# deeppowers/deeppowers

Measured on AMD Instinct MI355X. Metric: ciphertext-mul/s (N=4096, 4 RNS limbs), higher is better.
Workload: dtype u64

## Files before the change

### deeppowers_amd/csrc/devtables.h

```cpp
#pragma once
#include "modarith.h"

namespace dpfhe {

struct QuartersTop;

template <class Tw>
struct InvLast {
    Tw w_last;
    Tw w_ninv;
};

template <class Arith>
struct DevTables {
    const typename Arith::Tw* fwd;
    const typename Arith::Tw* inv;
    const typename Arith::Tw* fwd4;
    const typename Arith::Tw* inv4;
    const typename Arith::Tw* top_fwd;
    const typename Arith::Tw* top_inv;
    const InvLast<typename Arith::Tw>* top_last;
    int n_sub;
    const typename Arith::Tw* hfwd;
    const typename Arith::Tw* hinv;
    const typename Arith::Tw* htop_fwd;
    const InvLast<typename Arith::Tw>* htop_last;
    const typename Arith::Tw* qfwd;
    const typename Arith::Tw* qinv;
    const struct QuartersTop* qtop_fwd;
    const typename Arith::Tw* qtop_inv;
    const InvLast<typename Arith::Tw>* qtop_last;
    const InvLast<typename Arith::Tw>* last;
    const InvLast<typename Arith::Tw>* last2;
    const LimbConst* lc;
    int n_limbs;
    int n_active;
    unsigned long long active_map;
};

template <class TB>
DPF_HD void block_item_limb(const TB& tb, size_t blk, size_t& item, int& limb) {
    if (tb.n_active) {
        item = blk / (unsigned)tb.n_active;
        limb = (int)((tb.active_map >> (4u * (unsigned)(blk % (unsigned)tb.n_active))) & 15u);
    } else {
        item = blk / (unsigned)tb.n_limbs;
        limb = (int)(blk % (unsigned)tb.n_limbs);
    }
}

struct MixedTables {
    const void* fwd;
    const void* inv;
    const void* last;
    const LimbConst* lc;
    int n_limbs;
// ... 5 lines not shown
```

### deeppowers_amd/csrc/dpfhe_cabi.hip

```cpp
#include <dlfcn.h>
#include <hip/hip_runtime.h>

#include <algorithm>
#include <atomic>
#include <cstdio>
#include <cstdlib>
#include <cstring>
#include <mutex>
#include <new>
#include <string>
#include <type_traits>
#include <vector>

#include "../../include/dpfhe.h"
#include "base_ext.h"
#include "expand.h"
#include "plain_add.h"
#include "kernels_large.h"
#include "kernels_misc.h"
#include "launch.h"
#include "ntt_core.h"
#include "ntt_quarters.h"
#include "tables.h"

// ... 177 lines not shown
    return DPFHE_SUCCESS;
}
extern "C" int dpfhe_ctx_tune_info(const dpfhe_ctx* c, dpfhe_tune_info* out) {
    if (!c || !out) return fail(DPFHE_INVALID_ARGUMENT, "dpfhe_ctx_tune_info", "null argument");
    std::lock_guard<std::mutex> lk(c->tune_mutex);
    *out = c->tune;
    out->chosen = c->ct_mul_variant.load();
    return DPFHE_SUCCESS;
}
extern "C" int dpfhe_ctx_set_ct_mul_variant(dpfhe_ctx* c, int variant) {
    if (!c) return fail(DPFHE_INVALID_ARGUMENT, "dpfhe_ctx_set_ct_mul_variant", "null context");
    if (!ct_mul_variant_compiled(c, variant)) return fail(DPFHE_INVALID_ARGUMENT, "dpfhe_ctx_set_ct_mul_variant", "this context has no such form of the fused multiply");
    std::lock_guard<std::mutex> lk(c->tune_mutex);
    c->ct_mul_variant.store(variant);
    c->tune.chosen = variant;
    c->tune.source = DPFHE_TUNE_FORCED;
    return DPFHE_SUCCESS;
}
extern "C" const char* dpfhe_ct_mul_variant_name(int variant) {
    return variant >= 0 && variant < kCtMulVariants ? kCtMulVariantNames[variant] : "";
}

static_assert(sizeof(TwShoup) == 16 && sizeof(TwFold) == 16 && sizeof(TwF64) == 16, "the per-limb slots of the mixed tables share one stride");
struct MixedLayout { size_t o_lc, o_fwd4, o_inv4, o_fwd, o_inv, o_last, o_last2, total; };
static MixedLayout mixed_layout(int log2n, size_t L) {
    auto up = [](size_t x) { return (x + 255) & ~(size_t)255; };
    const size_t n = (size_t)1 << log2n, tab = L * n * 16;
    const bool two_geo = ntt_loge(log2n) != kFusedLoge;
    MixedLayout m;
    m.o_lc = 0; m.o_fwd4 = up(L * sizeof(LimbConst)); m.o_inv4 = up(m.o_fwd4 + tab);
    m.o_fwd = two_geo ? up(m.o_inv4 + tab) : m.o_fwd4; m.o_inv = two_geo ? up(m.o_fwd + tab) : m.o_inv4;
    m.o_last = up(m.o_inv + tab); m.o_last2 = up(m.o_last + L * 32); m.total = up(m.o_last2 + L * 32);
    return m;
}
template <class Tw, class MakeTw>
static void fill_mixed_limb(std::vector<unsigned char>& blob, const MixedLayout& m, int log2n, size_t l, const HostLimbTables& t, LimbClass cls, MakeTw make_tw) {
    static_assert(sizeof(Tw) == 16 && sizeof(InvLast<Tw>) == 32, "slot sizes");
    const size_t n = (size_t)1 << log2n;
    const u64 q = t.lc.q;
    const LimbConst lc = limb_const_of_class(t.lc, cls);
    std::memcpy(&blob[m.o_lc + l * sizeof(LimbConst)], &lc, sizeof(LimbConst));
    auto pack = [&](const std::vector<u64>& words, int loge, size_t off) {
        std::vector<Tw> tw(words.size());
        for (size_t i = 0; i < words.size(); ++i) tw[i] = make_tw(words[i], q);
        permute_window0(tw, log2n, loge, geo_perm_stages(log2n, loge));
        std::memcpy(&blob[off], tw.data(), tw.size() * sizeof(Tw));
    };
    pack(t.rp, kFusedLoge, m.o_fwd4 + l * n * 16);
    pack(t.irp, kFusedLoge, m.o_inv4 + l * n * 16);
    if (m.o_fwd != m.o_fwd4) { pack(t.rp, ntt_loge(log2n), m.o_fwd + l * n * 16); pack(t.irp, ntt_loge(log2n), m.o_inv + l * n * 16); }
    reinterpret_cast<InvLast<Tw>*>(&blob[m.o_last])[l] = InvLast<Tw>{make_tw(t.w_last, q), make_tw(t.lc.ninv, q)};
    const u64 sinv = cls == kClassFoldScaled ? h_powmod((1ull << fold_scaled_shift(q)) % q, q - 2, q) : 1;
    reinterpret_cast<InvLast<Tw>*>(&blob[m.o_last2])[l] = InvLast<Tw>{make_tw(h_mulmod(t.w_last, sinv, q), q), make_tw(h_mulmod(t.lc.ninv, sinv, q), q)};
}
template <class Arith>
static DevTables<Arith> mixed_view(const unsigned char* b, const MixedLayout& m, size_t L) {
    typedef typename Arith::Tw Tw;
    DevTables<Arith> tb{};
    tb.lc = reinterpret_cast<const LimbConst*>(b + m.o_lc);
    tb.fwd = reinterpret_cast<const Tw*>(b + m.o_fwd); tb.inv = reinterpret_cast<const Tw*>(b + m.o_inv);
    tb.fwd4 = reinterpret_cast<const Tw*>(b + m.o_fwd4); tb.inv4 = reinterpret_cast<const Tw*>(b + m.o_inv4);
    tb.last = reinterpret_cast<const InvLast<Tw>*>(b + m.o_last);
    tb.last2 = reinterpret_cast<const InvLast<Tw>*>(b + m.o_last2);
    tb.n_sub = 1;
    tb.n_limbs = (int)L;
    return tb;
}

extern "C" int dpfhe_ctx_create(dpfhe_ctx** out, uint32_t log2_n, uint32_t n_limbs, const uint64_t* moduli,
                                const uint64_t* psi, int device_id) {
    if (!out || !moduli || !psi) return fail(DPFHE_INVALID_ARGUMENT, "dpfhe_ctx_create", "null argument");
    if (log2_n < 8 || log2_n > (uint32_t)kMaxLog2N) return fail(DPFHE_INVALID_ARGUMENT, "dpfhe_ctx_create", "log2_n must be in [8, 16]");
    if (n_limbs == 0 || n_limbs > 1024) return fail(DPFHE_INVALID_ARGUMENT, "dpfhe_ctx_create", "n_limbs must be in [1, 1024]");
    const size_t n = (size_t)1 << log2_n, L = n_limbs;
    std::vector<HostLimbTables> ht(L);
    bool fold = true;
    for (size_t l = 0; l < L; ++l) {
        if (!h_is_prime(moduli[l])) return fail(DPFHE_INVALID_ARGUMENT, "dpfhe_ctx_create", "modulus is not prime");
        int rc = build_limb_tables((int)log2_n, moduli[l], psi[l], ht[l]);
        if (rc) return fail(rc, "dpfhe_ctx_create", "modulus must be < 2^60 and 1 mod 2N, psi a primitive 2N-th root");
        fold = fold && fold_eligible(moduli[l]);
    }
    int ndev = 0;
    HIP_TRY(hipGetDeviceCount(&ndev));
    if (device_id < 0 || device_id >= ndev) return fail(DPFHE_INVALID_ARGUMENT, "dpfhe_ctx_create", "no such device");
    int prev = 0;
// ... 3 lines not shown
    dpfhe_ctx* c = new (std::nothrow) dpfhe_ctx;
    if (!c) return fail(DPFHE_OUT_OF_MEMORY, "dpfhe_ctx_create", "host allocation");
    c->log2n = log2_n; c->n_limbs = n_limbs; c->device = device_id; c->fold = fold; c->p_special = moduli[L - 1];
    c->moduli.assign(moduli, moduli + L);
    { int cus = 0; if (hipDeviceGetAttribute(&cus, hipDeviceAttributeMultiprocessorCount, device_id) == hipSuccess && cus > 0) c->n_cu = cus; }

    auto up = [](size_t x) { return (x + 255) & ~(size_t)255; };
    const size_t tw_sz = fold ? sizeof(TwFold) : sizeof(TwShoup);
    const int log_n1 = split_log_n1((int)log2_n), log_n2 = (int)log2_n - log_n1;
    const size_t n_sub = (size_t)1 << log_n1, n2 = (size_t)1 << log_n2;
    const int loge_ntt = ntt_loge(log_n2);
    const bool split = log_n1 > 0, two_geo = !split && loge_ntt != kFusedLoge;
    const size_t tab = L * n * tw_sz;
    const size_t o_lc = 0, o_fwd4 = up(o_lc + L * sizeof(LimbConst)), o_inv4 = up(o_fwd4 + tab),
                 o_fwd = two_geo ? up(o_inv4 + tab) : o_fwd4, o_inv = two_geo ? up(o_fwd + tab) : o_inv4,
                 o_last = up(o_inv + tab), o_top_fwd = up(o_last + L * n_sub * 2 * tw_sz), o_top_inv = up(o_top_fwd + L * n_sub * tw_sz),
                 o_top_last = up(o_top_inv + L * n_sub * tw_sz), o_resc = up(o_top_last + L * 2 * tw_sz);
    const bool halves = log2_n == 13 && fold;
    const size_t o_hfwd = up(o_resc + L * sizeof(RescaleConst)), o_hinv = halves ? up(o_hfwd + tab) : o_hfwd, o_htop_fwd = halves ? up(o_hinv + tab) : o_hfwd,
                 o_htop_last = halves ? up(o_htop_fwd + L * tw_sz) : o_hfwd, o_q0 = halves ? up(o_htop_last + L * 2 * tw_sz) : o_hfwd;
    const bool quarters = log2_n == 14 && fold;
    const size_t o_qfwd = o_q0, o_qinv = quarters ? up(o_qfwd + tab) : o_q0, o_qtop_fwd = quarters ? up(o_qinv + tab) : o_q0,
                 o_qtop_inv = quarters ? up(o_qtop_fwd + L * sizeof(QuartersTop)) : o_q0, o_qtop_last = quarters ? up(o_qtop_inv + L * 2 * tw_sz) : o_q0,
                 total = quarters ? up(o_qtop_last + L * 2 * tw_sz) : o_q0;
    std::vector<unsigned char> blob(total, 0);
    auto fill = [&](auto tw_tag) {
        typedef decltype(tw_tag) Tw;
        for (size_t l = 0; l < L; ++l) {
            const u64 q = moduli[l];
            auto pack = [&](const std::vector<u64>& words, int logn_tab, int loge, size_t off) {
                std::vector<Tw> t(words.size());
                for (size_t i = 0; i < words.size(); ++i) t[i] = h_make_tw<Tw>(words[i], q);
                permute_window0(t, logn_tab, loge, geo_perm_stages(logn_tab, loge));
                std::memcpy(&blob[off], t.data(), t.size() * sizeof(Tw));
            };
            InvLast<Tw>* lasts = reinterpret_cast<InvLast<Tw>*>(&blob[o_last]);
            if (!split) {
                for (int geo = 0; geo < (two_geo ? 2 : 1); ++geo) {
                    const int loge = geo ? loge_ntt : kFusedLoge;
                    pack(ht[l].rp, (int)log2_n, loge, (geo ? o_fwd : o_fwd4) + l * n * tw_sz);
                    pack(ht[l].irp, (int)log2_n, loge, (geo ? o_inv : o_inv4) + l * n * tw_sz);
                }
                lasts[l] = InvLast<Tw>{h_make_tw<Tw>(ht[l].w_last, q), h_make_tw<Tw>(ht[l].lc.ninv, q)};
                if constexpr (std::is_same<Tw, TwFold>::value) {
                    if (quarters) {
                        for (size_t r = 0; r < 4; ++r) {
                            pack(subtree_table(ht[l].rp, 14, 2, r), 12, 4, o_qfwd + (l * 4 + r) * (n / 4) * tw_sz);
                            pack(subtree_table(ht[l].irp, 14, 2, r), 12, 4, o_qinv + (l * 4 + r) * (n / 4) * tw_sz);
                        }
                        reinterpret_cast<QuartersTop*>(&blob[o_qtop_fwd])[l] = QuartersTop{h_tw_fold(ht[l].rp[1], q), h_tw_fold(ht[l].rp[2], q), h_tw_fold(ht[l].rp[3], q)};
                        reinterpret_cast<TwFold*>(&blob[o_qtop_inv])[2 * l] = h_tw_fold(ht[l].irp[2], q);
                        reinterpret_cast<TwFold*>(&blob[o_qtop_inv])[2 * l + 1] = h_tw_fold(ht[l].irp[3], q);
                        reinterpret_cast<InvLast<TwFold>*>(&blob[o_qtop_last])[l] = InvLast<TwFold>{h_tw_fold(ht[l].w_last, q), h_tw_fold(ht[l].lc.ninv, q)};
                    }
                }
                if (halves) {
                    for (size_t r = 0; r < 2; ++r) {
                        pack(subtree_table(ht[l].rp, 13, 1, r), 12, 4, o_hfwd + (l * 2 + r) * (n / 2) * tw_sz);
                        pack(subtree_table(ht[l].irp, 13, 1, r), 12, 4, o_hinv + (l * 2 + r) * (n / 2) * tw_sz);
                    }
                    reinterpret_cast<Tw*>(&blob[o_htop_fwd])[l] = h_make_tw<Tw>(ht[l].rp[1], q);
                    reinterpret_cast<InvLast<Tw>*>(&blob[o_htop_last])[l] = lasts[l];
                }
            } else {
                for (size_t r = 0; r < n_sub; ++r) {
                    const std::vector<u64> f = subtree_table(ht[l].rp, (int)log2_n, log_n1, r), v = subtree_table(ht[l].irp, (int)log2_n, log_n1, r);
                    pack(f, log_n2, loge_ntt, o_fwd + (l * n_sub + r) * n2 * tw_sz);
// ... 21 lines not shown
    }
    hipError_t e = hipMalloc(&c->d_blob, total);
    if (e == hipSuccess) e = hipMemcpy(c->d_blob, blob.data(), total, hipMemcpyHostToDevice);
    if (e != hipSuccess) {
        if (c->d_blob) (void)hipFree(c->d_blob);
        delete c;
        (void)hipSetDevice(prev);
        return fail(e == hipErrorOutOfMemory ? DPFHE_OUT_OF_MEMORY : DPFHE_DEVICE_ERROR, "dpfhe_ctx_create: table upload", hipGetErrorString(e));
    }
    unsigned char* d = static_cast<unsigned char*>(c->d_blob);
    c->d_rescale = reinterpret_cast<const RescaleConst*>(d + o_resc);
    if (fold) {
        c->foldt.lc = reinterpret_cast<const LimbConst*>(d + o_lc);
        c->foldt.fwd = reinterpret_cast<const TwFold*>(d + o_fwd);
        c->foldt.inv = reinterpret_cast<const TwFold*>(d + o_inv);
        c->foldt.fwd4 = reinterpret_cast<const TwFold*>(d + o_fwd4);
        c->foldt.inv4 = reinterpret_cast<const TwFold*>(d + o_inv4);
        c->foldt.last = reinterpret_cast<const InvLast<TwFold>*>(d + o_last);
        c->foldt.top_fwd = reinterpret_cast<const TwFold*>(d + o_top_fwd);
        c->foldt.top_inv = reinterpret_cast<const TwFold*>(d + o_top_inv);
        c->foldt.top_last = reinterpret_cast<const InvLast<TwFold>*>(d + o_top_last);
        c->foldt.n_sub = (int)n_sub;
        c->foldt.n_limbs = (int)n_limbs;
        if (quarters) {
            c->foldt.qfwd = reinterpret_cast<const TwFold*>(d + o_qfwd); c->foldt.qinv = reinterpret_cast<const TwFold*>(d + o_qinv);
            c->foldt.qtop_fwd = reinterpret_cast<const QuartersTop*>(d + o_qtop_fwd); c->foldt.qtop_inv = reinterpret_cast<const TwFold*>(d + o_qtop_inv);
            c->foldt.qtop_last = reinterpret_cast<const InvLast<TwFold>*>(d + o_qtop_last);
        }
        if (halves) {
            c->foldt.hfwd = reinterpret_cast<const TwFold*>(d + o_hfwd); c->foldt.hinv = reinterpret_cast<const TwFold*>(d + o_hinv);
            c->foldt.htop_fwd = reinterpret_cast<const TwFold*>(d + o_htop_fwd); c->foldt.htop_last = reinterpret_cast<const InvLast<TwFold>*>(d + o_htop_last);
        }
    } else {
        c->shoup.lc = reinterpret_cast<const LimbConst*>(d + o_lc);
        c->shoup.fwd = reinterpret_cast<const TwShoup*>(d + o_fwd);
        c->shoup.inv = reinterpret_cast<const TwShoup*>(d + o_inv);
        c->shoup.fwd4 = reinterpret_cast<const TwShoup*>(d + o_fwd4);
        c->shoup.inv4 = reinterpret_cast<const TwShoup*>(d + o_inv4);
        c->shoup.last = reinterpret_cast<const InvLast<TwShoup>*>(d + o_last);
        c->shoup.top_fwd = reinterpret_cast<const TwShoup*>(d + o_top_fwd);
        c->shoup.top_inv = reinterpret_cast<const TwShoup*>(d + o_top_inv);
        c->shoup.top_last = reinterpret_cast<const InvLast<TwShoup>*>(d + o_top_last);
        c->shoup.n_sub = (int)n_sub;
        c->shoup.n_limbs = (int)n_limbs;
        if (halves) {
            c->shoup.hfwd = reinterpret_cast<const TwShoup*>(d + o_hfwd); c->shoup.hinv = reinterpret_cast<const TwShoup*>(d + o_hinv);
// ... 1302 lines not shown
```

### deeppowers_amd/csrc/kernels.h

```cpp
#pragma once
#include <hip/hip_runtime.h>

#include "devtables.h"
#include "launch.h"
#include "ntt_core.h"
#include "ntt_top.h"

namespace dpfhe {

__device__ __forceinline__ void lds_barrier() { __syncthreads(); }
__device__ __forceinline__ void wave_sync() {
    __builtin_amdgcn_fence(__ATOMIC_ACQ_REL, "wavefront");
    __builtin_amdgcn_wave_barrier();
}
template <class G, int X, bool FWD>
__device__ __forceinline__ void exch_sync_before_write() {
    if constexpr (G::exch_wave_local(X)) {
        wave_sync();
    } else {
        constexpr bool first = FWD ? X == 0 : G::highest_cross_wave_exchange() == X;
        if constexpr (!first) lds_barrier();
    }
}
template <class G, int X>
// ... 178 lines not shown
        if constexpr (P > 0) {
            exch_sync_before_write<typename B::G, P - 1, false>();
            B::template lds_write<P - 1, P, false>(tid, x, lds0);
            B::template inv_phase_r<P, IN>(y, twr, last.w_last, last.w_ninv, lc);
            B::template lds_write<P - 1, P, false>(tid, y, lds1);
            exch_sync_after_write<typename B::G, P - 1>();
            B::template lds_read<P - 1, P - 1, false>(tid, x, lds0);
            B::template lds_read<P - 1, P - 1, false>(tid, y, lds1);
            B::template inv_phase_r<P, IN>(z, twr, last.w_last, last.w_ninv, lc);
            TwRegs nxt;
            B::template load_tw<P - 1, false>(tid, tw, nxt);
            exch_sync_reuse<typename B::G, P - 1>();
            B::template lds_write<P - 1, P, false>(tid, z, lds0);
            exch_sync_after_write<typename B::G, P - 1>();
            B::template lds_read<P - 1, P - 1, false>(tid, z, lds0);
            InvChain3<B, P - 1, IN>::run_with(tid, x, y, z, lds0, lds1, tw, last, lc, nxt);
        } else {
            B::template inv_phase_r<P, IN>(y, twr, last.w_last, last.w_ninv, lc);
            B::template inv_phase_r<P, IN>(z, twr, last.w_last, last.w_ninv, lc);
        }
    }
};

template <class Arith, int LOGN, int LOGE, bool NT = false>
__global__ __launch_bounds__(1 << (LOGN - LOGE)) void ntt_fwd_kernel(u64* __restrict__ out, const u64* __restrict__ in,
                                                                      DevTables<Arith> tb) {
    typedef NttBody<Arith, LOGN, LOGE> B;
    __shared__ __attribute__((aligned(16))) u64 lds[B::G::lds_words()];
    const int tid = threadIdx.x;
    size_t p = blockIdx.x;
    const size_t sub = p % (size_t)tb.n_sub;
    int limb = (int)((p / (size_t)tb.n_sub) % (size_t)tb.n_limbs);
    if (tb.n_active) {
        size_t item;
        block_item_limb(tb, blockIdx.x, item, limb);
        p = item * (size_t)tb.n_limbs + (size_t)limb;
    }
    const LimbConst lc = tb.lc[limb];
    const typename B::Tw* tw = tb.fwd + ((size_t)limb * tb.n_sub + sub) * B::G::N;
    u64 x[B::E];
    B::template load_top<NT>(tid, x, in + p * B::G::N);
    FwdChain<B, 0>::run(tid, x, lds, tw, lc);
    B::fwd_canon(x, lc);
    if constexpr (B::kLdsIO) B::template store_bot_lds<NT>(tid, x, out + p * B::G::N, lds);
    else B::store_bot(tid, x, out + p * B::G::N);
}
// ... 282 lines not shown
        B::store_bot(tid, D2, dst + 2 * cstride);
    } else {
        asm volatile("" : "+v"(tid));
        InvChain2<BI, B::NPH - 1, kInvIn>::run(tid, D0, D1, lds, lds + W, twi, last, lc);
        B::inv_canon(D0, lc);
        B::template store_top<true>(tid, D0, dst);
        B::inv_canon(D1, lc);
        B::template store_top<true>(tid, D1, dst + cstride);
        asm volatile("" : "+v"(tid));
        lds_barrier();
        InvChain<BI, B::NPH - 1, kInvIn>::run(tid, D2, lds, twi, last, lc);
        B::inv_canon(D2, lc);
        B::template store_top<true>(tid, D2, dst + 2 * cstride);
    }
}

constexpr int kTraceWords = 12;
template <bool TRACE>
__device__ __forceinline__ u64 trace_stamp(u64 dep) {
    u64 t = 0;
    if constexpr (TRACE) asm volatile("s_memrealtime %0\n\ts_waitcnt lgkmcnt(0)" : "=s"(t) : "v"(dep) : "memory");
    return t;
}
template <class Arith, int LOGN, int LOGE, bool TRACE = false, bool OUT_NTT = false>
__global__ __launch_bounds__(1 << (LOGN - LOGE), 2) void ct_mul_quad_kernel(u64* __restrict__ out3, const u64* __restrict__ a2,
                                                                         const u64* __restrict__ b2, DevTables<Arith> tb, u64* __restrict__ trace = nullptr) {
    typedef NttBody<Arith, LOGN, LOGE> B;
    static_assert(B::kLazyProducts && LOGE == kFusedLoge, "a policy with lazy products (ntt_core.h prod), fused twiddle layout");
    typedef NttBody<Arith, LOGN, LOGE, 0, kUnit, true> BI;
    constexpr bool kScaledProducts = Arith::kFoldCore && !Arith::kFold;
    constexpr int E = B::E, N = B::G::N, W = B::G::lds_words();
    __shared__ __attribute__((aligned(16))) u64 lds[2 * W];
    const int tid = threadIdx.x;
    const u64 ts0 = trace_stamp<TRACE>((u64)tid);
    const size_t L = (size_t)tb.n_limbs;
    size_t bi;
    int limb;
    block_item_limb(tb, blockIdx.x, bi, limb);
    const LimbConst lc = tb.lc[limb];
    const u64* src_a = a2 + ((bi * 2) * L + limb) * N;
    const u64* src_b = b2 + ((bi * 2) * L + limb) * N;
    u64* dst = out3 + ((bi * 3) * L + limb) * N;
    const size_t cstride = L * N;
    const InvLast<typename B::Tw> last = kScaledProducts ? tb.last2[limb] : tb.last[limb];
    constexpr int kInvIn = B::kProdInvIn;
    u64 x[E], y[E], z[E], w[E];
    const u64 ts_p = trace_stamp<TRACE>((u64)(uintptr_t)src_a ^ (u64)lc.q);
// ... 5 lines not shown
    const u64 ts_i = trace_stamp<TRACE>((u64)tid);
    const u64 ts1 = trace_stamp<TRACE>(x[0]);
    const u64 ts_xl = trace_stamp<TRACE>(x[E - 1]);
    FwdChain4<B, 0>::run(tid, x, y, z, w, lds, lds + W, tb.fwd4 + (size_t)limb * N, lc);
    B::prod_partner(y, lc);
    B::prod_partner(w, lc);
    const u64 ts2 = trace_stamp<TRACE>(w[E - 1]);
#pragma unroll
    for (int k = 0; k < E; ++k) {
        const u64 a0 = x[k], b0 = y[k], a1 = z[k], b1 = w[k];
        B::tensor(a0, a1, b0, b1, x[k], y[k], z[k], lc);
    }
    const u64 ts3 = trace_stamp<TRACE>(z[E - 1]);
    if constexpr (OUT_NTT) {
        static_assert(Arith::kFold && !TRACE, "the pinned primes (the products of a scaled-fold limb carry the scale twice)");
#pragma unroll
        for (int k = 0; k < E; ++k) { x[k] = FoldArith::canon_small(x[k], lc); y[k] = FoldArith::canon_small(y[k], lc); z[k] = FoldArith::canon_small(z[k], lc); }
        B::store_bot(tid, x, dst);
        B::store_bot(tid, y, dst + cstride);
        B::store_bot(tid, z, dst + 2 * cstride);
        return;
    }
    constexpr bool kNtStore = true;
    InvChain3<BI, B::NPH - 1, kInvIn>::run(tid, x, y, z, lds, lds + W, tb.inv4 + (size_t)limb * N, last, lc);
    const u64 ts4 = trace_stamp<TRACE>(z[E - 1]);
    B::inv_canon(x, lc);
    B::template store_top<kNtStore>(tid, x, dst);
    B::inv_canon(y, lc);
    B::template store_top<kNtStore>(tid, y, dst + cstride);
    B::inv_canon(z, lc);
    B::template store_top<kNtStore>(tid, z, dst + 2 * cstride);
    if constexpr (TRACE) {
        const u64 ts5 = trace_stamp<TRACE>((u64)tid);
        asm volatile("s_waitcnt vmcnt(0)" ::: "memory");
        const u64 ts6 = trace_stamp<TRACE>((u64)tid);
        if (tid == 0) {
            unsigned hw, xcc;
            asm volatile("s_getreg_b32 %0, hwreg(HW_REG_HW_ID)" : "=s"(hw));
            asm volatile("s_getreg_b32 %0, hwreg(HW_REG_XCC_ID)" : "=s"(xcc));
            u64* t = trace + (size_t)blockIdx.x * kTraceWords;
            t[0] = ts0; t[1] = ts1; t[2] = ts2; t[3] = ts3; t[4] = ts4; t[5] = ts5; t[6] = ts6;
            t[7] = (u64)hw | ((u64)xcc << 32);
            t[8] = ts_p; t[9] = ts_x; t[10] = ts_i; t[11] = ts_xl;
        }
    }
}

constexpr unsigned kRelinRotMajor = 0x80000000u;
template <class Arith>
__device__ __forceinline__ u64 canon_any(u64 v, const LimbConst& lc) {
    if (Arith::kFold) return FoldArith::canon(v, lc);
    else return ShoupArith::mul_var(v, 1, lc);
}

// ... 401 lines not shown
```

### deeppowers_amd/csrc/launch_impl.h

```cpp
#pragma once
#include <cstdlib>

#include "kernels.h"
#include "launch.h"
#include "kernels_halves.h"
#include "kernels_quarters.h"
#ifdef DPFHE_DIAGNOSTICS
#include "kernels_trace.h"
#endif

namespace dpfhe {

constexpr size_t kLdsBytesPerCu = 160 * 1024;
static_assert(2 * sizeof(u64) * Geo<13, kFusedLoge>::lds_words() <= kLdsBytesPerCu, "two LDS images of an N = 8192 polynomial must fit one CU's 160 KiB");
static_assert(2 * sizeof(u64) * Geo<13, kFusedLoge>::lds_words() == 163840 && 2 * sizeof(u64) * Geo<12, kFusedLoge>::lds_words() == 77824,
              "LDS footprint of the paired fused kernels changed: re-check the 160 KiB budget at N = 8192 (zero margin) and two workgroups per CU at N = 4096");
static_assert(sizeof(u64) * Geo<14, 4>::lds_words() <= kLdsBytesPerCu, "the N = 16384 transform's LDS image must fit one CU's 160 KiB");

#define DPFHE_GEO_SWITCH(log2n, MACRO) \
    switch (log2n) {                   \
        case 8: MACRO(8, 4); break;    \
        case 9: MACRO(9, 4); break;    \
        case 10: MACRO(10, 4); break;  \
        case 11: MACRO(11, 4); break;  \
// ... 73 lines not shown
            return 0;
        }
    }
#define NTT_CASE(LN, LE)                                                                                                              \
    if constexpr (Arith::kFold && (LN == 12 || LN == 13)) {                                                                           \
        if (nt) {                                                                                                                     \
            if (inverse) hipLaunchKernelGGL((ntt_inv_kernel<Arith, LN, LE, true>), dim3((unsigned)npolys), dim3(Geo<LN, LE>::T), 0, s, out, in, tb); \
            else hipLaunchKernelGGL((ntt_fwd_kernel<Arith, LN, LE, true>), dim3((unsigned)npolys), dim3(Geo<LN, LE>::T), 0, s, out, in, tb);         \
            break;                                                                                                                    \
        }                                                                                                                             \
    }                                                                                                                                 \
    if (inverse) hipLaunchKernelGGL((ntt_inv_kernel<Arith, LN, LE>), dim3((unsigned)npolys), dim3(Geo<LN, LE>::T), 0, s, out, in, tb); \
    else hipLaunchKernelGGL((ntt_fwd_kernel<Arith, LN, LE>), dim3((unsigned)npolys), dim3(Geo<LN, LE>::T), 0, s, out, in, tb)
    DPFHE_NTT_GEO_SWITCH(log2n, NTT_CASE)
#undef NTT_CASE
    return 0;
}

template <class Arith, bool IN_NTT, bool OUT_NTT>
static int launch_ct_mul_dom(int log2n, u64* out3, const u64* a2, const u64* b2, size_t blocks, const DevTables<Arith>& tb, hipStream_t s) {
    constexpr int kQuadMaxLogN = 12, kDualMaxLogN = 13;
#define CT_CASE(LN, LE)                                                                                                                              \
    if constexpr (Arith::kFoldCore && !IN_NTT && !OUT_NTT && LN <= kQuadMaxLogN)                                              \
        hipLaunchKernelGGL((ct_mul_quad_kernel<Arith, LN, kFusedLoge>), dim3((unsigned)blocks), dim3(Geo<LN, kFusedLoge>::T), 0, s, out3, a2, b2, tb, (u64*)nullptr); \
    else if constexpr (Arith::kFold && !IN_NTT && OUT_NTT && LN <= kQuadMaxLogN)    \
        hipLaunchKernelGGL((ct_mul_quad_kernel<Arith, LN, kFusedLoge, false, true>), dim3((unsigned)blocks), dim3(Geo<LN, kFusedLoge>::T), 0, s, out3, a2, b2, tb, (u64*)nullptr); \
    else if constexpr ((Arith::kFoldCore || Arith::kF64) && !IN_NTT && LN <= kDualMaxLogN)                                                                                                     \
        hipLaunchKernelGGL((ct_mul_dual_kernel<Arith, LN, kFusedLoge, OUT_NTT>), dim3((unsigned)blocks), dim3(Geo<LN, kFusedLoge>::T), 0, s, out3, a2, b2, tb); \
    else                                                                                                                                             \
        hipLaunchKernelGGL((ct_mul_kernel<Arith, LN, kFusedLoge, IN_NTT, OUT_NTT>), dim3((unsigned)blocks), dim3(Geo<LN, kFusedLoge>::T), 0, s, out3, a2, b2, tb)
    DPFHE_GEO_SWITCH(log2n, CT_CASE)
#undef CT_CASE
    return 0;
}

template <class Arith>
int launch_ct_mul(int log2n, unsigned flags, u64* out3, const u64* a2, const u64* b2, size_t blocks, const DevTables<Arith>& tb, hipStream_t s) {
    switch (flags & 3u) {
        case 0: return launch_ct_mul_dom<Arith, false, false>(log2n, out3, a2, b2, blocks, tb, s);
        case 1: return launch_ct_mul_dom<Arith, true, false>(log2n, out3, a2, b2, blocks, tb, s);
        case 2: return launch_ct_mul_dom<Arith, false, true>(log2n, out3, a2, b2, blocks, tb, s);
        default: return launch_ct_mul_dom<Arith, true, true>(log2n, out3, a2, b2, blocks, tb, s);
    }
}

template <class Arith>
int launch_ct_mul_variant(int log2n, int variant, u64* out3, const u64* a2, const u64* b2, size_t blocks, const DevTables<Arith>& tb, hipStream_t s) {
    if constexpr (!Arith::kFold) return -1;
    else {
#define CTV_CASE(LN)                                                                                                                                  \
    case LN:                                                                                                                                          \
        if (variant == kCtMulQuad) hipLaunchKernelGGL((ct_mul_quad_kernel<Arith, LN, kFusedLoge>), dim3((unsigned)blocks), dim3(Geo<LN, kFusedLoge>::T), 0, s, out3, a2, b2, tb, (u64*)nullptr); \
        else if (variant == kCtMulDual) hipLaunchKernelGGL((ct_mul_dual_kernel<Arith, LN, kFusedLoge, false>), dim3((unsigned)blocks), dim3(Geo<LN, kFusedLoge>::T), 0, s, out3, a2, b2, tb); \
        else return -1;                                                                                                                               \
        return 0
        switch (log2n) {
            CTV_CASE(12);
            CTV_CASE(13);
            default: return -1;
        }
#undef CTV_CASE
    }
}
template <class Arith>
int launch_ct_mul_trace(int log2n, u64* out3, const u64* a2, const u64* b2, size_t blocks, const DevTables<Arith>& tb, u64* trace, hipStream_t s) {
    if constexpr (!Arith::kFold) return -1;
    else {
        if (log2n != 12) return -1;
        hipLaunchKernelGGL((ct_mul_quad_kernel<Arith, 12, kFusedLoge, true>), dim3((unsigned)blocks), dim3(Geo<12, kFusedLoge>::T), 0, s, out3, a2, b2, tb, trace);
        return 0;
    }
}

#ifdef DPFHE_DIAGNOSTICS
inline u64* g_relin_trace = nullptr;
inline unsigned g_relin_trace_blocks = 0;
#endif
template <class Arith>
int launch_relin(int log2n, int mode, u64* out2, const u64* in3, const u64* evk, size_t key_stride, unsigned key_group, size_t blocks,
                 const DevTables<Arith>& tb, hipStream_t s) {
    if (mode < 0 || mode > 4) return -1;
    const unsigned La = tb.n_active ? (unsigned)tb.n_active : (unsigned)tb.n_limbs;
    const int n_digits = mode >= 2 ? tb.n_limbs - 1 : tb.n_limbs;
    const unsigned kg = key_group ? key_group : 1u;
    unsigned n_outer = ((kg > 1 || key_stride != 0) && blocks % ((size_t)kg * La) == 0) ? (unsigned)(blocks / kg) : 0u;
    unsigned grid = n_outer ? ((n_outer + 7u) / 8u) * 8u * kg : (unsigned)blocks;
    if (n_outer && n_outer / La >= 8u) {
        const unsigned n_keys = n_outer / La;
        grid = ((n_keys + 7u) / 8u) * 8u * La * kg;
        n_outer |= kRelinRotMajor;
    }
#ifdef DPFHE_DIAGNOSTICS
// ... 72 lines not shown
```

### deeppowers_amd/csrc/ntt_core.h

```cpp
#pragma once
#include "modarith.h"

namespace dpfhe {

#if defined(DPFHE_EMU_CHECK) && !defined(__HIPCC__)
inline u64 chk_add(u64 a, u64 b) { if ((unsigned __int128)a + b >> 64) ++g_emu_overflows; return a + b; }
inline u64 chk_sub_add(u64 a, u64 b, u64 off) {
    __int128 v = (__int128)a - (__int128)b + (__int128)off;
    if (v < 0 || (v >> 64)) ++g_emu_overflows;
    return a - b + off;
}
inline u64 chk_shl1_add_sub(u64 a, u64 c, u64 s) {
    __int128 v = 2 * (__int128)a + (__int128)c - (__int128)s;
    if (v < 0 || (v >> 64) || ((unsigned __int128)2 * a + c) >> 64) ++g_emu_overflows;
    return shl1_add(a, c) - s;
}
#else
DPF_HD u64 chk_shl1_add_sub(u64 a, u64 c, u64 s) { return shl1_add(a, c) - s; }
DPF_HD u64 chk_add(u64 a, u64 b) { return a + b; }
DPF_HD u64 chk_sub_add(u64 a, u64 b, u64 off) { return a - b + off; }
#endif

struct Phase {
    int c;
// ... 147 lines not shown
};

template <int LOGE>
constexpr CtfPlan<LOGE> make_ctf_plan(int lb_top, int r, int in_bound, int out_cap) {
    CtfPlan<LOGE> p{};
    constexpr int E = 1 << LOGE;
    int bnd[E] = {};
    for (int k = 0; k < E; ++k) bnd[k] = in_bound;
    for (int u = 0; u < r; ++u) {
        const int bit = 1 << (lb_top - u);
        for (int k = 0; k < E; ++k) {
            if (k & bit) continue;
            int A = bnd[k];
            const int Y = bnd[k | bit];
            if (A + Y / 4 + 1 > kFuseLimit || (u == r - 1 && A > kRedB && 2 * A + 2 * kUnit > out_cap)) { p.red_a[u][k] = true; A = kRedB; }
            bnd[k] = kRedB;
            bnd[k | bit] = 2 * A + 2 * kUnit;
        }
    }
    int mx = 0;
    for (int k = 0; k < E; ++k) {
        if (bnd[k] > out_cap) { p.red_end[k] = true; bnd[k] = kRedB; }
        p.out[k] = bnd[k];
        if (bnd[k] > mx) mx = bnd[k];
    }
    p.out_bound = mx;
    return p;
}

constexpr int kF64Red = kUnit / 2 + 1, kF64Tw = kUnit;
template <int LOGE>
struct F64CtPlan {
    bool red_y[LOGE][1 << LOGE];
    bool red_a[LOGE][1 << LOGE];
    bool red_end[1 << LOGE];
    int out_bound;
};
template <int LOGE>
constexpr F64CtPlan<LOGE> make_f64_ct_plan(int lb_top, int r, int in_bound, int out_cap, int cap) {
    F64CtPlan<LOGE> p{};
    constexpr int E = 1 << LOGE;
    int bnd[E] = {};
    for (int k = 0; k < E; ++k) bnd[k] = in_bound;
    for (int u = 0; u < r; ++u) {
        const int bit = 1 << (lb_top - u);
        for (int k = 0; k < E; ++k) {
// ... 554 lines not shown
    }
    static DPF_HD u64 tw_mul(u64 y, const Tw& t, const LimbConst& lc) {
        if constexpr (Arith::kFoldCore) return FoldArith::mul_tw(y, t, lc);
        else return Arith::mul_tw(y, t, lc);
    }
    template <int P, int IN>
    static DPF_HD void inv_phase(int tid, u64 (&x)[E], const Tw* tw, const Tw& w_last, const Tw& w_ninv, const LimbConst& lc) {
        TwRegs twr;
        load_tw<P, false>(tid, tw, twr);
        inv_phase_r<P, IN>(x, twr, w_last, w_ninv, lc);
    }
    static_assert(!Arith::kFold || SUB || (kWord >> LOGN) + 2 <= kUnit / 2, "the exact division's output (make_gs_plan: kUnit + (sum >> LOGN) + 2) must fit canon_small");
    static DPF_HD void inv_canon(u64 (&x)[E], const LimbConst& lc_in) {
        const auto& lc = Arith::ntt_lc(lc_in);
#pragma clang loop unroll(full)
        for (int k = 0; k < E; ++k) {
            if constexpr (Arith::kF64) x[k] = Arith::leave(x[k], lc);
            else if constexpr (Arith::kFoldCore) {
                x[k] = FoldArith::canon_small(x[k], lc);
                if constexpr (kConverts) x[k] = Arith::leave(x[k], lc_in);
            } else x[k] = csub(x[k], lc.q);
        }
    }
};

}
```

### deeppowers_amd/csrc/tables.h

```cpp
#pragma once
#include <vector>

#include "modarith.h"

namespace dpfhe {

typedef unsigned __int128 u128;

inline u64 h_mulmod(u64 a, u64 b, u64 q) { return (u64)((u128)a * b % q); }
inline u64 h_powmod(u64 b, u64 e, u64 q) {
    u64 r = 1;
    b %= q;
    for (; e; e >>= 1) {
        if (e & 1) r = h_mulmod(r, b, q);
        b = h_mulmod(b, b, q);
    }
    return r;
}
inline bool h_is_prime(u64 n) {
    if (n < 2) return false;
    const u64 bases[12] = {2, 3, 5, 7, 11, 13, 17, 19, 23, 29, 31, 37};
    for (u64 p : bases) {
        if (n == p) return true;
        if (n % p == 0) return false;
// ... 70 lines not shown
    for (size_t m = 1; m < n2; m <<= 1)
        for (size_t i = 0; i < m; ++i) sub[m + i] = table[root * m + i];
    return sub;
}

inline bool fold_eligible(u64 q) { return q < (1ull << 60) && ((1ull << 60) - q) < (1ull << 24); }

template <class Tw>
inline void permute_window0(std::vector<Tw>& t, int log2n, int loge, int perm_stages) {
    const size_t n = (size_t)1 << log2n, T = n >> loge;
    std::vector<Tw> src(t);
    for (int pos = 0; pos < perm_stages && pos < loge - 1; ++pos) {
        const size_t m = n >> (pos + 1), cnt = m / T;
        for (size_t tid = 0; tid < T; ++tid)
            for (size_t i = 0; i < cnt; ++i) t[m + i * T + tid] = src[m + tid * cnt + i];
    }
}

struct HostLimbTables {
    LimbConst lc;
    std::vector<u64> rp, irp;
    std::vector<u64> rp_sh, irp_sh;
    u64 w_last, w_last_sh;
};

inline int build_limb_tables(int log2n, u64 q, u64 psi, HostLimbTables& t) {
    const u64 n = 1ull << log2n;
    if (log2n < 1 || log2n > 20) return 2000;
    if (q < 3 || (q >> 60) || (q - 1) % (2 * n) != 0) return 2000;
    if (psi == 0 || psi >= q || h_powmod(psi, n, q) != q - 1) return 2000;
    t.rp.assign(n, 0); t.irp.assign(n, 0); t.rp_sh.assign(n, 0); t.irp_sh.assign(n, 0);
    const u64 ipsi = h_powmod(psi, q - 2, q);
    u64 pw = 1, ipw = 1;
    for (u64 i = 0; i < n; ++i) {
        const u32 r = h_brv((u32)i, log2n);
        t.rp[r] = pw; t.rp_sh[r] = h_shoup(pw, q);
        t.irp[r] = ipw; t.irp_sh[r] = h_shoup(ipw, q);
        pw = h_mulmod(pw, psi, q); ipw = h_mulmod(ipw, ipsi, q);
    }
    LimbConst& c = t.lc;
    c.q = q;
    c.d = fold_eligible(q) ? (1ull << 60) - q : 0;
    c.ninv = h_powmod(n % q, q - 2, q);
    c.ninv_sh = h_shoup(c.ninv, q);
    const u128 ratio = (~(u128)0) / q;
    c.br_hi = (u64)(ratio >> 64); c.br_lo = (u64)ratio;
    c.two64 = (u64)((((u128)1) << 64) % q);
    c.pad1 = 0;
    t.w_last = h_mulmod(t.irp[1], c.ninv, q);
    t.w_last_sh = h_shoup(t.w_last, q);
    return 0;
}

}
```

Measured before the change: 2.385 million.

## Use cyclic inverse NTT with post-twist in fused ciphertext multiply

Replaces the negacyclic inverse NTT in the quad ct-mul kernel with a cyclic Cooley-Tukey inverse using trivial-twiddle butterflies in window 0. It then applies a per-coefficient post-twist that folds in psi^-j and N^-1, replacing the separate last-stage scaling. The aim is fewer modular multiplies in the inverse chain. In exchange it adds an N-entry twist table per limb that must be loaded from global memory, plus extra table memory, and the path is restricted to fold-class primes.

```diff
diff --git a/deeppowers_amd/csrc/devtables.h b/deeppowers_amd/csrc/devtables.h
--- a/deeppowers_amd/csrc/devtables.h
+++ b/deeppowers_amd/csrc/devtables.h
@@ -32,6 +32,8 @@
     const InvLast<typename Arith::Tw>* qtop_last;
     const InvLast<typename Arith::Tw>* last;
     const InvLast<typename Arith::Tw>* last2;
+    const typename Arith::Tw* ctinv;
+    const typename Arith::Tw* twist;
     const LimbConst* lc;
     int n_limbs;
     int n_active;
diff --git a/deeppowers_amd/csrc/dpfhe_cabi.hip b/deeppowers_amd/csrc/dpfhe_cabi.hip
--- a/deeppowers_amd/csrc/dpfhe_cabi.hip
+++ b/deeppowers_amd/csrc/dpfhe_cabi.hip
@@ -223,7 +223,7 @@
 }
 
 static_assert(sizeof(TwShoup) == 16 && sizeof(TwFold) == 16 && sizeof(TwF64) == 16, "the per-limb slots of the mixed tables share one stride");
-struct MixedLayout { size_t o_lc, o_fwd4, o_inv4, o_fwd, o_inv, o_last, o_last2, total; };
+struct MixedLayout { size_t o_lc, o_fwd4, o_inv4, o_fwd, o_inv, o_last, o_last2, o_ctinv, o_twist, total; };
 static MixedLayout mixed_layout(int log2n, size_t L) {
     auto up = [](size_t x) { return (x + 255) & ~(size_t)255; };
     const size_t n = (size_t)1 << log2n, tab = L * n * 16;
@@ -231,7 +231,9 @@
     MixedLayout m;
     m.o_lc = 0; m.o_fwd4 = up(L * sizeof(LimbConst)); m.o_inv4 = up(m.o_fwd4 + tab);
     m.o_fwd = two_geo ? up(m.o_inv4 + tab) : m.o_fwd4; m.o_inv = two_geo ? up(m.o_fwd + tab) : m.o_inv4;
-    m.o_last = up(m.o_inv + tab); m.o_last2 = up(m.o_last + L * 32); m.total = up(m.o_last2 + L * 32);
+    m.o_last = up(m.o_inv + tab); m.o_last2 = up(m.o_last + L * 32);
+    const bool ct = log2n <= kMaxFusedLog2N;
+    m.o_ctinv = up(m.o_last2 + L * 32); m.o_twist = ct ? up(m.o_ctinv + tab) : m.o_ctinv; m.total = ct ? up(m.o_twist + tab) : m.o_ctinv;
     return m;
 }
 template <class Tw, class MakeTw>
@@ -253,6 +255,11 @@
     reinterpret_cast<InvLast<Tw>*>(&blob[m.o_last])[l] = InvLast<Tw>{make_tw(t.w_last, q), make_tw(t.lc.ninv, q)};
     const u64 sinv = cls == kClassFoldScaled ? h_powmod((1ull << fold_scaled_shift(q)) % q, q - 2, q) : 1;
     reinterpret_cast<InvLast<Tw>*>(&blob[m.o_last2])[l] = InvLast<Tw>{make_tw(h_mulmod(t.w_last, sinv, q), q), make_tw(h_mulmod(t.lc.ninv, sinv, q), q)};
+    if (cls == kClassFold && m.o_twist != m.o_ctinv) {
+        Tw* tc = reinterpret_cast<Tw*>(&blob[m.o_ctinv]) + l * n;
+        Tw* tt = reinterpret_cast<Tw*>(&blob[m.o_twist]) + l * n;
+        for (size_t i = 0; i < n; ++i) { tc[i] = make_tw(t.ctw[i], q); tt[i] = make_tw(t.twist[i], q); }
+    }
 }
 template <class Arith>
 static DevTables<Arith> mixed_view(const unsigned char* b, const MixedLayout& m, size_t L) {
@@ -263,6 +270,7 @@
     tb.fwd4 = reinterpret_cast<const Tw*>(b + m.o_fwd4); tb.inv4 = reinterpret_cast<const Tw*>(b + m.o_inv4);
     tb.last = reinterpret_cast<const InvLast<Tw>*>(b + m.o_last);
     tb.last2 = reinterpret_cast<const InvLast<Tw>*>(b + m.o_last2);
+    if (m.o_twist != m.o_ctinv) { tb.ctinv = reinterpret_cast<const Tw*>(b + m.o_ctinv); tb.twist = reinterpret_cast<const Tw*>(b + m.o_twist); }
     tb.n_sub = 1;
     tb.n_limbs = (int)L;
     return tb;
@@ -312,7 +320,9 @@
     const bool quarters = log2_n == 14 && fold;
     const size_t o_qfwd = o_q0, o_qinv = quarters ? up(o_qfwd + tab) : o_q0, o_qtop_fwd = quarters ? up(o_qinv + tab) : o_q0,
                  o_qtop_inv = quarters ? up(o_qtop_fwd + L * sizeof(QuartersTop)) : o_q0, o_qtop_last = quarters ? up(o_qtop_inv + L * 2 * tw_sz) : o_q0,
-                 total = quarters ? up(o_qtop_last + L * 2 * tw_sz) : o_q0;
+                 o_ct0 = quarters ? up(o_qtop_last + L * 2 * tw_sz) : o_q0;
+    const bool ct_tabs = fold && !split && log2_n <= (uint32_t)kMaxFusedLog2N;
+    const size_t o_ctinv = o_ct0, o_twist = ct_tabs ? up(o_ctinv + tab) : o_ct0, total = ct_tabs ? up(o_twist + tab) : o_ct0;
     std::vector<unsigned char> blob(total, 0);
     auto fill = [&](auto tw_tag) {
         typedef decltype(tw_tag) Tw;
@@ -333,6 +343,11 @@
                 }
                 lasts[l] = InvLast<Tw>{h_make_tw<Tw>(ht[l].w_last, q), h_make_tw<Tw>(ht[l].lc.ninv, q)};
                 if constexpr (std::is_same<Tw, TwFold>::value) {
+                    if (ct_tabs) {
+                        TwFold* tc = reinterpret_cast<TwFold*>(&blob[o_ctinv]) + l * n;
+                        TwFold* tt = reinterpret_cast<TwFold*>(&blob[o_twist]) + l * n;
+                        for (size_t i = 0; i < n; ++i) { tc[i] = h_tw_fold(ht[l].ctw[i], q); tt[i] = h_tw_fold(ht[l].twist[i], q); }
+                    }
                     if (quarters) {
                         for (size_t r = 0; r < 4; ++r) {
                             pack(subtree_table(ht[l].rp, 14, 2, r), 12, 4, o_qfwd + (l * 4 + r) * (n / 4) * tw_sz);
@@ -400,6 +415,7 @@
         c->foldt.top_last = reinterpret_cast<const InvLast<TwFold>*>(d + o_top_last);
         c->foldt.n_sub = (int)n_sub;
         c->foldt.n_limbs = (int)n_limbs;
+        if (ct_tabs) { c->foldt.ctinv = reinterpret_cast<const TwFold*>(d + o_ctinv); c->foldt.twist = reinterpret_cast<const TwFold*>(d + o_twist); }
         if (quarters) {
             c->foldt.qfwd = reinterpret_cast<const TwFold*>(d + o_qfwd); c->foldt.qinv = reinterpret_cast<const TwFold*>(d + o_qinv);
             c->foldt.qtop_fwd = reinterpret_cast<const QuartersTop*>(d + o_qtop_fwd); c->foldt.qtop_inv = reinterpret_cast<const TwFold*>(d + o_qtop_inv);
diff --git a/deeppowers_amd/csrc/kernels.h b/deeppowers_amd/csrc/kernels.h
--- a/deeppowers_amd/csrc/kernels.h
+++ b/deeppowers_amd/csrc/kernels.h
@@ -224,6 +224,43 @@
     }
 };
 
+template <class B, int P, int IN>
+struct InvChain3Ct {
+    typedef typename B::TwRegs TwRegs;
+    typedef typename B::Tw Tw;
+    static __device__ __forceinline__ void run(int tid, u64 (&x)[B::E], u64 (&y)[B::E], u64 (&z)[B::E], u64* lds0, u64* lds1, const Tw* tw,
+                                               const Tw* twist, Tw (&t)[B::E], const LimbConst& lc) {
+        TwRegs twr;
+        B::template load_ct_tw<P>(tid, tw, twr);
+        run_with(tid, x, y, z, lds0, lds1, tw, twist, t, lc, twr);
+    }
+    static __device__ __forceinline__ void run_with(int tid, u64 (&x)[B::E], u64 (&y)[B::E], u64 (&z)[B::E], u64* lds0, u64* lds1,
+                                                    const Tw* tw, const Tw* twist, Tw (&t)[B::E], const LimbConst& lc, const TwRegs& twr) {
+        B::template ct_inv_phase_r<P, IN>(x, twr, lc);
+        if constexpr (P > 0) {
+            exch_sync_before_write<typename B::G, P - 1, false>();
+            B::template lds_write<P - 1, P, false>(tid, x, lds0);
+            B::template ct_inv_phase_r<P, IN>(y, twr, lc);
+            B::template lds_write<P - 1, P, false>(tid, y, lds1);
+            exch_sync_after_write<typename B::G, P - 1>();
+            B::template lds_read<P - 1, P - 1, false>(tid, x, lds0);
+            B::template lds_read<P - 1, P - 1, false>(tid, y, lds1);
+            B::template ct_inv_phase_r<P, IN>(z, twr, lc);
+            TwRegs nxt;
+            B::template load_ct_tw<P - 1>(tid, tw, nxt);
+            exch_sync_reuse<typename B::G, P - 1>();
+            B::template lds_write<P - 1, P, false>(tid, z, lds0);
+            exch_sync_after_write<typename B::G, P - 1>();
+            B::template lds_read<P - 1, P - 1, false>(tid, z, lds0);
+            InvChain3Ct<B, P - 1, IN>::run_with(tid, x, y, z, lds0, lds1, tw, twist, t, lc, nxt);
+        } else {
+            B::load_twist(tid, twist, t);
+            B::template ct_inv_phase_r<P, IN>(y, twr, lc);
+            B::template ct_inv_phase_r<P, IN>(z, twr, lc);
+        }
+    }
+};
+
 template <class Arith, int LOGN, int LOGE, bool NT = false>
 __global__ __launch_bounds__(1 << (LOGN - LOGE)) void ntt_fwd_kernel(u64* __restrict__ out, const u64* __restrict__ in,
                                                                       DevTables<Arith> tb) {
@@ -552,7 +589,7 @@
     if constexpr (TRACE) asm volatile("s_memrealtime %0\n\ts_waitcnt lgkmcnt(0)" : "=s"(t) : "v"(dep) : "memory");
     return t;
 }
-template <class Arith, int LOGN, int LOGE, bool TRACE = false, bool OUT_NTT = false>
+template <class Arith, int LOGN, int LOGE, bool TRACE = false, bool OUT_NTT = false, bool CT_INV = false>
 __global__ __launch_bounds__(1 << (LOGN - LOGE), 2) void ct_mul_quad_kernel(u64* __restrict__ out3, const u64* __restrict__ a2,
                                                                          const u64* __restrict__ b2, DevTables<Arith> tb, u64* __restrict__ trace = nullptr) {
     typedef NttBody<Arith, LOGN, LOGE> B;
@@ -604,14 +641,28 @@
         return;
     }
     constexpr bool kNtStore = true;
-    InvChain3<BI, B::NPH - 1, kInvIn>::run(tid, x, y, z, lds, lds + W, tb.inv4 + (size_t)limb * N, last, lc);
-    const u64 ts4 = trace_stamp<TRACE>(z[E - 1]);
-    B::inv_canon(x, lc);
-    B::template store_top<kNtStore>(tid, x, dst);
-    B::inv_canon(y, lc);
-    B::template store_top<kNtStore>(tid, y, dst + cstride);
-    B::inv_canon(z, lc);
-    B::template store_top<kNtStore>(tid, z, dst + 2 * cstride);
+    u64 ts4 = 0;
+    if constexpr (CT_INV) {
+        static_assert(Arith::kFold, "the pinned primes (the cyclic inverse's post-twist replaces the exact division by N)");
+        typename B::Tw t[E];
+        InvChain3Ct<BI, B::NPH - 1, kInvIn>::run(tid, x, y, z, lds, lds + W, tb.ctinv + (size_t)limb * N, tb.twist + (size_t)limb * N, t, lc);
+        ts4 = trace_stamp<TRACE>(z[E - 1]);
+        B::twist_canon(x, t, lc);
+        B::template store_top<kNtStore>(tid, x, dst);
+        B::twist_canon(y, t, lc);
+        B::template store_top<kNtStore>(tid, y, dst + cstride);
+        B::twist_canon(z, t, lc);
+        B::template store_top<kNtStore>(tid, z, dst + 2 * cstride);
+    } else {
+        InvChain3<BI, B::NPH - 1, kInvIn>::run(tid, x, y, z, lds, lds + W, tb.inv4 + (size_t)limb * N, last, lc);
+        ts4 = trace_stamp<TRACE>(z[E - 1]);
+        B::inv_canon(x, lc);
+        B::template store_top<kNtStore>(tid, x, dst);
+        B::inv_canon(y, lc);
+        B::template store_top<kNtStore>(tid, y, dst + cstride);
+        B::inv_canon(z, lc);
+        B::template store_top<kNtStore>(tid, z, dst + 2 * cstride);
+    }
     if constexpr (TRACE) {
         const u64 ts5 = trace_stamp<TRACE>((u64)tid);
         asm volatile("s_waitcnt vmcnt(0)" ::: "memory");
diff --git a/deeppowers_amd/csrc/launch_impl.h b/deeppowers_amd/csrc/launch_impl.h
--- a/deeppowers_amd/csrc/launch_impl.h
+++ b/deeppowers_amd/csrc/launch_impl.h
@@ -119,7 +119,7 @@
     constexpr int kQuadMaxLogN = 12, kDualMaxLogN = 13;
 #define CT_CASE(LN, LE)                                                                                                                              \
     if constexpr (Arith::kFoldCore && !IN_NTT && !OUT_NTT && LN <= kQuadMaxLogN)                                              \
-        hipLaunchKernelGGL((ct_mul_quad_kernel<Arith, LN, kFusedLoge>), dim3((unsigned)blocks), dim3(Geo<LN, kFusedLoge>::T), 0, s, out3, a2, b2, tb, (u64*)nullptr); \
+        hipLaunchKernelGGL((ct_mul_quad_kernel<Arith, LN, kFusedLoge, false, false, Arith::kFold>), dim3((unsigned)blocks), dim3(Geo<LN, kFusedLoge>::T), 0, s, out3, a2, b2, tb, (u64*)nullptr); \
     else if constexpr (Arith::kFold && !IN_NTT && OUT_NTT && LN <= kQuadMaxLogN)    \
         hipLaunchKernelGGL((ct_mul_quad_kernel<Arith, LN, kFusedLoge, false, true>), dim3((unsigned)blocks), dim3(Geo<LN, kFusedLoge>::T), 0, s, out3, a2, b2, tb, (u64*)nullptr); \
     else if constexpr ((Arith::kFoldCore || Arith::kF64) && !IN_NTT && LN <= kDualMaxLogN)                                                                                                     \
@@ -147,7 +147,7 @@
     else {
 #define CTV_CASE(LN)                                                                                                                                  \
     case LN:                                                                                                                                          \
-        if (variant == kCtMulQuad) hipLaunchKernelGGL((ct_mul_quad_kernel<Arith, LN, kFusedLoge>), dim3((unsigned)blocks), dim3(Geo<LN, kFusedLoge>::T), 0, s, out3, a2, b2, tb, (u64*)nullptr); \
+        if (variant == kCtMulQuad) hipLaunchKernelGGL((ct_mul_quad_kernel<Arith, LN, kFusedLoge, false, false, Arith::kFold>), dim3((unsigned)blocks), dim3(Geo<LN, kFusedLoge>::T), 0, s, out3, a2, b2, tb, (u64*)nullptr); \
         else if (variant == kCtMulDual) hipLaunchKernelGGL((ct_mul_dual_kernel<Arith, LN, kFusedLoge, false>), dim3((unsigned)blocks), dim3(Geo<LN, kFusedLoge>::T), 0, s, out3, a2, b2, tb); \
         else return -1;                                                                                                                               \
         return 0
@@ -164,7 +164,7 @@
     if constexpr (!Arith::kFold) return -1;
     else {
         if (log2n != 12) return -1;
-        hipLaunchKernelGGL((ct_mul_quad_kernel<Arith, 12, kFusedLoge, true>), dim3((unsigned)blocks), dim3(Geo<12, kFusedLoge>::T), 0, s, out3, a2, b2, tb, trace);
+        hipLaunchKernelGGL((ct_mul_quad_kernel<Arith, 12, kFusedLoge, true, false, Arith::kFold>), dim3((unsigned)blocks), dim3(Geo<12, kFusedLoge>::T), 0, s, out3, a2, b2, tb, trace);
         return 0;
     }
 }
diff --git a/deeppowers_amd/csrc/ntt_core.h b/deeppowers_amd/csrc/ntt_core.h
--- a/deeppowers_amd/csrc/ntt_core.h
+++ b/deeppowers_amd/csrc/ntt_core.h
@@ -193,6 +193,52 @@
     for (int k = 0; k < E; ++k) {
         if (bnd[k] > out_cap) { p.red_end[k] = true; bnd[k] = kRedB; }
         p.out[k] = bnd[k];
+        if (bnd[k] > mx) mx = bnd[k];
+    }
+    p.out_bound = mx;
+    return p;
+}
+
+template <int LOGE>
+struct CtiPlan {
+    bool triv[LOGE][1 << LOGE];
+    bool red_a[LOGE][1 << LOGE];
+    bool red_y[LOGE][1 << LOGE];
+    int off[LOGE][1 << LOGE];
+    bool red_end[1 << LOGE];
+    int out_bound;
+};
+template <int LOGE>
+constexpr CtiPlan<LOGE> make_cti_plan(int lb0, int r, bool window0, int in_bound, int out_cap) {
+    CtiPlan<LOGE> p{};
+    constexpr int E = 1 << LOGE;
+    int bnd[E] = {};
+    for (int k = 0; k < E; ++k) bnd[k] = in_bound;
+    for (int u = 0; u < r; ++u) {
+        const int bit = 1 << (lb0 + u);
+        for (int k = 0; k < E; ++k) {
+            if (k & bit) continue;
+            int A = bnd[k], Y = bnd[k | bit];
+            if (window0 && (k & (bit - 1)) == 0) {
+                p.triv[u][k] = true;
+                while (A + (Y + kUnit - 1) / kUnit * kUnit > kWord || A + Y > kWord) {
+                    if (Y >= A && Y > kRedB) { p.red_y[u][k] = true; Y = kRedB; }
+                    else { p.red_a[u][k] = true; A = kRedB; }
+                }
+                const int offq = (Y + kUnit - 1) / kUnit;
+                p.off[u][k] = offq;
+                bnd[k] = A + Y;
+                bnd[k | bit] = A + offq * kUnit;
+            } else {
+                if (A + Y / 4 + 1 > kFuseLimit || (u == r - 1 && A > kRedB && 2 * A + 2 * kUnit > out_cap)) { p.red_a[u][k] = true; A = kRedB; }
+                bnd[k] = kRedB;
+                bnd[k | bit] = 2 * A + 2 * kUnit;
+            }
+        }
+    }
+    int mx = 0;
+    for (int k = 0; k < E; ++k) {
+        if (bnd[k] > out_cap) { p.red_end[k] = true; bnd[k] = kRedB; }
         if (bnd[k] > mx) mx = bnd[k];
     }
     p.out_bound = mx;
@@ -793,6 +839,76 @@
             } else x[k] = csub(x[k], lc.q);
         }
     }
+
+    template <int P>
+    static DPF_HD void load_ct_tw(int tid, const Tw* tw, TwRegs& twr) {
+        constexpr Phase ph = G::phase(P);
+        const unsigned tl = (ph.c + LOGE >= LOGN) ? (unsigned)tid : ((unsigned)tid & ((1u << ph.c) - 1u));
+#pragma clang loop unroll(full)
+        for (int u = 0; u < ph.r; ++u) {
+            const int pos = ph.b + u, lb = pos - ph.c;
+#pragma clang loop unroll(full)
+            for (int i = 0; i < E / 2; ++i) {
+                if (i >= (1 << lb) || (ph.c == 0 && i == 0)) continue;
+                if (ph.c == 0) twr[u][i] = tw[(1 << pos) + i];
+                else twr[u][i] = (tw + (1 << pos) + (i << ph.c))[tl];
+            }
+        }
+    }
+    template <int P, int IN>
+    static constexpr CtiPlan<LOGE> cti_plan() {
+        constexpr Phase ph = G::phase(P);
+        int in = IN;
+        for (int i = NPH - 1; i > P; --i) {
+            const Phase pi = G::phase(i);
+            in = make_cti_plan<LOGE>(pi.b - pi.c, pi.r, pi.c == 0, in, kCtfMid).out_bound;
+        }
+        return make_cti_plan<LOGE>(ph.b - ph.c, ph.r, ph.c == 0, in, P == 0 ? kWord : kCtfMid);
+    }
+    template <int P, int IN>
+    static DPF_HD void ct_inv_phase_r(u64 (&x)[E], const TwRegs& twr, const LimbConst& lc) {
+        static_assert(Arith::kFold, "the pinned primes: the post-twist replaces the exact division by N");
+        constexpr Phase ph = G::phase(P);
+        constexpr CtiPlan<LOGE> plan = cti_plan<P, IN>();
+        const u64 two_q = 2 * lc.q;
+#pragma clang loop unroll(full)
+        for (int u = 0; u < ph.r; ++u) {
+            const int lb = ph.b + u - ph.c;
+#pragma clang loop unroll(full)
+            for (int k = 0; k < E; ++k) {
+                if (k & (1 << lb)) continue;
+                const int kk = k | (1 << lb);
+                u64 a = x[k], y = x[kk];
+                if (plan.red_a[u][k]) a = FoldArith::reduce(a, lc);
+                if (plan.triv[u][k]) {
+                    if (plan.red_y[u][k]) y = FoldArith::reduce(y, lc);
+                    x[k] = chk_add(a, y);
+                    x[kk] = chk_sub_add(a, y, (u64)plan.off[u][k] * lc.q);
+                } else {
+                    const u64 s = FoldArith::mul_tw_add(y, twr[u][k & ((1 << lb) - 1)], lc, a);
+                    x[k] = s;
+                    x[kk] = chk_shl1_add_sub(a, two_q, s);
+                }
+            }
+        }
+#pragma clang loop unroll(full)
+        for (int k = 0; k < E; ++k)
+            if (plan.red_end[k]) x[k] = FoldArith::reduce(x[k], lc);
+    }
+    template <int P, int IN>
+    static DPF_HD void ct_inv_phase(int tid, u64 (&x)[E], const Tw* tw, const LimbConst& lc) {
+        TwRegs twr;
+        load_ct_tw<P>(tid, tw, twr);
+        ct_inv_phase_r<P, IN>(x, twr, lc);
+    }
+    static DPF_HD void load_twist(int tid, const Tw* twist, Tw (&t)[E]) {
+#pragma clang loop unroll(full)
+        for (int k = 0; k < E; ++k) t[k] = (twist + k * T)[(unsigned)tid];
+    }
+    static DPF_HD void twist_canon(u64 (&x)[E], const Tw (&t)[E], const LimbConst& lc) {
+#pragma clang loop unroll(full)
+        for (int k = 0; k < E; ++k) x[k] = FoldArith::canon_small(FoldArith::mul_tw(x[k], t[k], lc), lc);
+    }
 };
 
 }
diff --git a/deeppowers_amd/csrc/tables.h b/deeppowers_amd/csrc/tables.h
--- a/deeppowers_amd/csrc/tables.h
+++ b/deeppowers_amd/csrc/tables.h
@@ -116,6 +116,7 @@
     std::vector<u64> rp, irp;
     std::vector<u64> rp_sh, irp_sh;
     u64 w_last, w_last_sh;
+    std::vector<u64> ctw, twist;
 };
 
 inline int build_limb_tables(int log2n, u64 q, u64 psi, HostLimbTables& t) {
@@ -143,6 +144,14 @@
     c.pad1 = 0;
     t.w_last = h_mulmod(t.irp[1], c.ninv, q);
     t.w_last_sh = h_shoup(t.w_last, q);
+    t.ctw.assign(n, 0); t.twist.assign(n, 0);
+    const u64 iomega = h_mulmod(ipsi, ipsi, q);
+    for (u64 h = 1; h < n; h <<= 1) {
+        const u64 step = h_powmod(iomega, n / (2 * h), q);
+        u64 w = 1;
+        for (u64 i = 0; i < h; ++i) { t.ctw[h + i] = w; w = h_mulmod(w, step, q); }
+    }
+    for (u64 j = 0, w = c.ninv; j < n; ++j) { t.twist[j] = w; w = h_mulmod(w, ipsi, q); }
     return 0;
 }
 
```

Result: faster. 2.447 million, median of 6 (+2.6%).
